# stevenmiller888/mlx-audio

Measured on AMD Instinct MI355X. Metric: audio-sec/sec (xRT), Kokoro-82M batch=32 fixed 128-phoneme utterances per GPU, higher is better.
Workload: dtype bf16; 1 GPU; Kokoro-82M bf16, batch=32/GPU fixed 128-phoneme utterances (T=130, F=650, 390000 samples = 16.25 s each), utterance-sharded over 1 GPU(s); global_batch=32, parallelism=utterance-shard x1, 2 batches in flight per GPU

## Files before the change

### mlx-audio_amd/csrc/kk_conv_mfma4.hip

```cpp
#include <stdlib.h>

#include "kk_common.h"
#include "kk_kernels.h"
#include "kk_conv_mfma_shared.h"

#define TR_NOW() 0ull
#define TR_ADD(slot, v) do { } while (0)
namespace {
typedef __bf16 bf16x2 __attribute__((ext_vector_type(2)));

typedef __bf16 bf16x8 __attribute__((ext_vector_type(8)));
typedef float f32x4 __attribute__((ext_vector_type(4)));

constexpr int BN = 128, CK = 64;
constexpr int XLD = 80;
constexpr int MAX_HALO = 50;
constexpr int CLD = BN;

constexpr int PS_BYTES = 2 * 3 * CK * 4;

template <int BM>
struct Geo {
  static constexpr int XROWS = BM + MAX_HALO;
  static constexpr int XS_BYTES = XROWS * XLD * 2;
  static constexpr int MAIN_BYTES = XS_BYTES + PS_BYTES;
  static constexpr int RPP = BM / 2;
  static constexpr int EPI_BYTES = RPP * CLD * 4;
  static constexpr int LDS_BYTES = MAIN_BYTES > EPI_BYTES ? MAIN_BYTES : EPI_BYTES;
  static constexpr int XREG = (XROWS * 8 + 255) / 256;
};


union U16 {
  uint4 u;
  bf16_t h[8];
};
union U32x8 {
  uint4 u[2];
  float f[8];
};

template <typename TO, int WM, int NRM>
__global__ __launch_bounds__(256, 2) __attribute__((amdgpu_waves_per_eu(2, 2))) void conv_mfma4_kernel(KKMfmaArgs a) {
  constexpr int BM = 2 * WM, MI16 = WM / 16;
  constexpr bool ACC16 = true;
  using G = Geo<BM>;
  constexpr int XREG = G::XREG;
  extern __shared__ __attribute__((aligned(16))) unsigned char smem[];
  bf16_t* Xs = (bf16_t*)smem;
  float* Ps = (float*)(smem + G::XS_BYTES);
  float* Cs = (float*)smem;

  const int tid = threadIdx.x, lane = tid & 63, wave = tid >> 6;
  const int wr = wave >> 1, wc = wave & 1;
  const int nphase = a.mode == KK_CONVT ? a.stride : 1;
  int bx, by, bz;
  {
    const int gx = gridDim.x, gy = gridDim.y, total = gx * gy * gridDim.z;
    int lid = blockIdx.x + gx * (blockIdx.y + gy * blockIdx.z);
    const int per = total / 8, rem = total - per * 8;
    const int xcd = lid & 7, idx = lid >> 3;
    lid = xcd * per + (xcd < rem ? xcd : rem) + idx;
    by = lid % gy;
    const int t = lid / gy;
    bx = t % gx;
    bz = t / gx;
  }
  const int b = bz / nphase, phase = bz - b * nphase;
  const int q0 = bx * BM, n0 = by * BN;
  const int Lin = kk_len(a.lin, b), Lout = kk_len(a.lout, b);

  int ntaps, off0, dstep, widx0, wstep;
  if (a.mode == KK_CONV) {
    ntaps = a.Kw; off0 = -a.pad; dstep = a.dil; widx0 = 0; wstep = 1;
  } else {
    const int k0 = (phase + a.pad) % a.stride;
    ntaps = (a.Kw - k0 + a.stride - 1) / a.stride;
    off0 = (phase + a.pad - k0) / a.stride; dstep = -1; widx0 = k0; wstep = a.stride;
  }
  const int min_off = dstep >= 0 ? off0 : off0 + (ntaps - 1) * dstep;
  const int halo = (ntaps - 1) * (dstep >= 0 ? dstep : -dstep);
  const int xrows = BM + halo;

  const int op_first = a.mode == KK_CONV ? q0 : phase + a.stride * q0;
  const bool tile_live = op_first < Lout;

  const unsigned long long tr0 = TR_NOW();
  unsigned long long tr_sx = 0, tr_sw = 0;
  (void)tr0; (void)tr_sx; (void)tr_sw;
  f32x4 acc[MI16][4];
#pragma unroll
  for (int i = 0; i < MI16; ++i)
#pragma unroll
    for (int j = 0; j < 4; ++j) acc[i][j] = f32x4{0.f, 0.f, 0.f, 0.f};

  if (tile_live) {
    const bf16_t* xb = a.x + (long long)b * a.xbs;
    const int nchunk = a.CinP / CK;
    const int nit = nchunk * ntaps;
    const int lin_hi = Lin > 0 ? Lin - 1 : 0;
    const int cin_real = a.Cin > 0 ? a.Cin : a.CinP;

#define KK_STG(name) name
#define KK_STG_XS Xs
#include "kk_conv_mfma_stage.h"
    uint4 q00, q01, q02, q03, q10, q11, q12, q13;
    const int nb = by;
    auto frag_ptr = [&](int it) __attribute__((always_inline)) -> const uint4* {
      const int chunk = it / ntaps, tap = it - chunk * ntaps;
      const long long blk = ((long long)(widx0 + tap * wstep) * (a.CoutP / BN) + nb) * nchunk + chunk;
      return (const uint4*)a.wf + blk * 1024 + (wc * 2) * 4 * 64 + lane;
    };
    load_x(0);
    {
      const uint4* fp = frag_ptr(0);
      q00 = fp[0 * 64]; q01 = fp[1 * 64]; q02 = fp[2 * 64]; q03 = fp[3 * 64];
      q10 = fp[4 * 64]; q11 = fp[5 * 64]; q12 = fp[6 * 64]; q13 = fp[7 * 64];
      asm volatile("" ::: "memory");
    }
    store_p(0);
    __syncthreads();
    store_x(0);
    __syncthreads();

    const int arow = wr * WM + (lane & 15);
    const int kofs = 8 * (lane >> 4);

    for (int it = 0; it < nit; ++it) {
      const int chunk = it / ntaps, tap = it - chunk * ntaps;
      const bool last_tap = tap == ntaps - 1;
      if (tap == 0 && chunk + 1 < nchunk) load_x(chunk + 1);
      const uint4* fn = frag_ptr(it + 1 < nit ? it + 1 : it);

      const int shift = (off0 + tap * dstep) - min_off;
      const bf16_t* xa = Xs + (arow + shift) * XLD + kofs;
      KK_MFMA_ITER(q00, q01, q02, q03, q10, q11, q12, q13)
      asm volatile("" ::: "memory");
      if (it + 1 < nit) {
        if (tap == 0 && chunk + 1 < nchunk) store_p(chunk + 1);
        if (last_tap) {
          __syncthreads();
          store_x(chunk + 1);
          __syncthreads();
        }
      }
    }
    __syncthreads();
  }

#include "kk_conv_mfma_epilogue.h"
}

template <int XR>
struct GeoWK {
  static constexpr int SROWS = XR == 7 ? 224 : 192 + MAX_HALO;
  static constexpr int SLAB = SROWS * XLD;
  static constexpr int XS_BYTES = 2 * SLAB * 2;
  static constexpr int MAIN_BYTES = XS_BYTES + PS_BYTES;
  static constexpr int RPP = 96;
  static constexpr int EPI_BYTES = RPP * CLD * 4;
  static constexpr int LDS_BYTES = MAIN_BYTES > EPI_BYTES ? MAIN_BYTES : EPI_BYTES;
};

template <int NRM, int XR>
__global__ __launch_bounds__(256, 2) __attribute__((amdgpu_waves_per_eu(2, 2))) void conv_mfma4_wholek_kernel(KKMfmaArgs a) {
  using TO = bf16_t;
  constexpr int WM = 96, BM = 2 * WM, MI16 = WM / 16, XREG = XR;
  constexpr bool ACC16 = true;
  using G = GeoWK<XR>;
  extern __shared__ __attribute__((aligned(16))) unsigned char smem[];
  bf16_t* Xs = (bf16_t*)smem;
  float* Ps = (float*)(smem + G::XS_BYTES);
  float* Cs = (float*)smem;

  const int tid = threadIdx.x, lane = tid & 63, wave = tid >> 6;
  const int wr = wave >> 1, wc = wave & 1;
  constexpr int nphase = 1, phase = 0;
  int bx, by, b;
  {
    const int gx = gridDim.x, gy = gridDim.y, total = gx * gy * gridDim.z;
    int lid = blockIdx.x + gx * (blockIdx.y + gy * blockIdx.z);
    const int per = total / 8, rem = total - per * 8;
    const int xcd = lid & 7, idx = lid >> 3;
    lid = xcd * per + (xcd < rem ? xcd : rem) + idx;
    by = lid % gy;
    const int t = lid / gy;
    bx = t % gx;
    b = t / gx;
  }
  const int q0 = bx * BM, n0 = by * BN;
  const int Lin = kk_len(a.lin, b), Lout = kk_len(a.lout, b);
  const int ntaps = a.Kw, off0 = -a.pad, dstep = a.dil, min_off = off0;
  const int xrows = BM + (ntaps - 1) * dstep;
  const bool tile_live = q0 < Lout;

  const unsigned long long tr0 = TR_NOW();
  (void)tr0;
  f32x4 acc[MI16][4];
#pragma unroll
  for (int i = 0; i < MI16; ++i)
#pragma unroll
    for (int j = 0; j < 4; ++j) acc[i][j] = f32x4{0.f, 0.f, 0.f, 0.f};

  if (tile_live) {
    const bf16_t* xb = a.x + (long long)b * a.xbs;
    const int nit = 2 * ntaps;
    const int lin_hi = Lin > 0 ? Lin - 1 : 0;
    const int cin_real = a.Cin > 0 ? a.Cin : a.CinP;

#define KK_STG(name) name##_s0
#define KK_STG_XS Xs
#include "kk_conv_mfma_stage.h"
#define KK_STG(name) name##_s1
#define KK_STG_XS (Xs + G::SLAB)
#include "kk_conv_mfma_stage.h"
    uint4 q00, q01, q02, q03, q10, q11, q12, q13;
    auto frag_ptr = [&](int it) __attribute__((always_inline)) -> const uint4* {
      const int chunk = it >= ntaps ? 1 : 0, tap = it - chunk * ntaps;
      const long long blk = ((long long)tap * (a.CoutP / BN) + by) * 2 + chunk;
      return (const uint4*)a.wf + blk * 1024 + (wc * 2) * 4 * 64 + lane;
    };
    load_x_s0(0);
    load_x_s1(1);
    {
      const uint4* fp = frag_ptr(0);
      q00 = fp[0 * 64]; q01 = fp[1 * 64]; q02 = fp[2 * 64]; q03 = fp[3 * 64];
      q10 = fp[4 * 64]; q11 = fp[5 * 64]; q12 = fp[6 * 64]; q13 = fp[7 * 64];
      asm volatile("" ::: "memory");
    }
    store_p_s0(0);
    store_p_s1(1);
    __syncthreads();
    store_x_s0(0);
    store_x_s1(1);
    __syncthreads();

    const int arow = wr * WM + (lane & 15);
    const int kofs = 8 * (lane >> 4);
    for (int it = 0; it + 1 < nit; ++it) {
      const int chunk = it >= ntaps ? 1 : 0, tap = it - chunk * ntaps;
      const uint4* fn = frag_ptr(it + 1);
      const bf16_t* xa = Xs + chunk * G::SLAB + (arow + tap * dstep) * XLD + kofs;
      KK_MFMA_ITER(q00, q01, q02, q03, q10, q11, q12, q13)
      asm volatile("" ::: "memory");
    }
    {
      const bf16_t* xa = Xs + G::SLAB + (arow + (ntaps - 1) * dstep) * XLD + kofs;
      KK_MFMA_ITER_LAST(q00, q01, q02, q03, q10, q11, q12, q13)
      asm volatile("" ::: "memory");
    }
    __syncthreads();
  }

#include "kk_conv_mfma_epilogue.h"
}

template <int NRM, int XR>
int launch_wholek(const KKMfmaArgs& a, int B, hipStream_t st) {
  using G = GeoWK<XR>;
  static KKDevOnce attr_once;
  if (attr_once.first()) {
    (void)hipFuncSetAttribute((const void*)conv_mfma4_wholek_kernel<NRM, XR>, hipFuncAttributeMaxDynamicSharedMemorySize, G::LDS_BYTES);
    attr_once.done();
  }
  dim3 grid(kk_cdiv(a.Q, 192), a.CoutP / BN, B);
  hipLaunchKernelGGL((conv_mfma4_wholek_kernel<NRM, XR>), grid, dim3(256), G::LDS_BYTES, st, a);
  KK_CHECK_LAUNCH();
  return 0;
}

template <typename TO, int WM, int NRM>
int launch_one(const KKMfmaArgs& a, int B, hipStream_t st) {
  using G = Geo<2 * WM>;
  static KKDevOnce attr_once;
  if (attr_once.first()) {
    (void)hipFuncSetAttribute((const void*)conv_mfma4_kernel<TO, WM, NRM>, hipFuncAttributeMaxDynamicSharedMemorySize, G::LDS_BYTES);
    attr_once.done();
  }
  const int nphase = a.mode == KK_CONVT ? a.stride : 1;
  dim3 grid(kk_cdiv(a.Q, 2 * WM), a.CoutP / BN, B * nphase);
  hipLaunchKernelGGL((conv_mfma4_kernel<TO, WM, NRM>), grid, dim3(256), G::LDS_BYTES, st, a);
  KK_CHECK_LAUNCH();
  return 0;
}

__global__ __launch_bounds__(256) void pack_w_frag_kernel(const bf16_t* w, bf16_t* wf, int Kw, int CoutP, int CinP) {
  const long long n = (long long)Kw * CoutP * CinP;
  for (long long e = (long long)blockIdx.x * 256 + threadIdx.x; e < n; e += (long long)gridDim.x * 256) {
    const int k = (int)(e % CinP);
    const long long r = e / CinP;
    const int cout = (int)(r % CoutP), tap = (int)(r / CoutP);
    wf[KK_MFMA4_PACK_INDEX(tap, cout, k, CoutP, CinP)] = w[e];
  }
}
}

int kk_launch_pack_w_frag(const void* w, void* wf, int Kw, int CoutP, int CinP, hipStream_t st) {
  if (CinP % CK != 0 || CoutP % BN != 0) return kk_fail("pack_w_frag: CinP must be a multiple of 64 and CoutP of 128");
  hipLaunchKernelGGL(pack_w_frag_kernel, dim3(1024), dim3(256), 0, st, (const bf16_t*)w, (bf16_t*)wf, Kw, CoutP, CinP);
  KK_CHECK_LAUNCH();
  return 0;
}

bool kk_mfma4_wholek_eligible(const KKMfmaArgs& a) {
  return a.mode == KK_CONV && a.stride == 1 && a.CinP == 2 * CK && a.dil >= 1 && (a.Kw - 1) * a.dil <= MAX_HALO;
}

int kk_launch_conv_mfma4(const KKMfmaArgs& a, int B, int out_dtype, hipStream_t st) {
  if (a.Q <= 0 || B <= 0) return 0;
  if (!a.wf) return kk_fail("conv_mfma4: fragment-order weights missing");
  const int nrm = a.nrm_a == nullptr ? 0 : (a.nrm_act == KK_ACT_SNAKE ? 1 : 2);
  if (nrm == 1 && a.nrm_C % 4 != 0) return kk_fail("conv_mfma: the fused Snake input needs a channel count that is a multiple of 4");
  KKMfmaArgs g = a;
  if (nrm == 2 && a.nrm_act != KK_ACT_LRELU) g.nrm_slope = 1.0f;
  if (out_dtype != KK_BF16) return kk_fail("conv_mfma4: bf16 output only");
  if (kk_mfma4_wholek_eligible(g) && !g.slabwise) {
    const bool x7 = (g.Kw - 1) * g.dil <= 32;
    if (nrm == 1) return x7 ? launch_wholek<1, 7>(g, B, st) : launch_wholek<1, 8>(g, B, st);
    if (nrm == 2) return x7 ? launch_wholek<2, 7>(g, B, st) : launch_wholek<2, 8>(g, B, st);
    return x7 ? launch_wholek<0, 7>(g, B, st) : launch_wholek<0, 8>(g, B, st);
  }
  if (nrm == 1) return launch_one<bf16_t, 96, 1>(g, B, st);
  if (nrm == 2) return launch_one<bf16_t, 96, 2>(g, B, st);
  return launch_one<bf16_t, 96, 0>(g, B, st);
}
```

### mlx-audio_amd/csrc/kk_conv_mfma_shared.h

```cpp
#pragma once
#include <hip/hip_runtime.h>

namespace {
struct v2f {
  float x, y;
};
__device__ __forceinline__ v2f operator*(v2f a, v2f b) { return v2f{a.x * b.x, a.y * b.y}; }
__device__ __forceinline__ v2f& operator+=(v2f& a, v2f b) { a.x += b.x; a.y += b.y; return a; }
__device__ __forceinline__ v2f& operator*=(v2f& a, v2f b) { a.x *= b.x; a.y *= b.y; return a; }
__device__ __forceinline__ v2f fma2(v2f a, v2f b, v2f c) { return v2f{__builtin_fmaf(a.x, b.x, c.x), __builtin_fmaf(a.y, b.y, c.y)}; }
__device__ __forceinline__ float gelu_exact(float v) { return 0.5f * v * (1.0f + erff(v * 0.70710678118654752440f)); }

typedef float kk_f32x4 __attribute__((ext_vector_type(4)));
typedef __bf16 kk_bf16x8 __attribute__((ext_vector_type(8)));

#define KK_MFMA_KSTEP(KS, B0, B1, B2, B3)                                                                                                  \
  {                                                                                                                                          \
    const kk_bf16x8 b0 = __builtin_bit_cast(kk_bf16x8, B0), b1 = __builtin_bit_cast(kk_bf16x8, B1);                                          \
    const kk_bf16x8 b2 = __builtin_bit_cast(kk_bf16x8, B2), b3 = __builtin_bit_cast(kk_bf16x8, B3);                                          \
    _Pragma("unroll") for (int mi = 0; mi < MI16; ++mi) {                                                                                    \
      const kk_bf16x8 av = *(const kk_bf16x8*)(xa + mi * 16 * XLD + (KS) * 32);                                                              \
      acc[mi][0] = __builtin_amdgcn_mfma_f32_16x16x32_bf16(av, b0, acc[mi][0], 0, 0, 0);                                                     \
      acc[mi][1] = __builtin_amdgcn_mfma_f32_16x16x32_bf16(av, b1, acc[mi][1], 0, 0, 0);                                                     \
      acc[mi][2] = __builtin_amdgcn_mfma_f32_16x16x32_bf16(av, b2, acc[mi][2], 0, 0, 0);                                                     \
      acc[mi][3] = __builtin_amdgcn_mfma_f32_16x16x32_bf16(av, b3, acc[mi][3], 0, 0, 0);                                                     \
    }                                                                                                                                        \
    B0 = fn[((KS) * 4 + 0) * 64];                                                                                                            \
    B1 = fn[((KS) * 4 + 1) * 64];                                                                                                            \
    B2 = fn[((KS) * 4 + 2) * 64];                                                                                                            \
    B3 = fn[((KS) * 4 + 3) * 64];                                                                                                            \
  }
#define KK_MFMA_ITER(Q00, Q01, Q02, Q03, Q10, Q11, Q12, Q13)                                                                               \
  KK_MFMA_KSTEP(0, Q00, Q01, Q02, Q03)                                                                                                     \
  KK_MFMA_KSTEP(1, Q10, Q11, Q12, Q13)                                                                                                     \
  __builtin_amdgcn_sched_group_barrier(0x100, 2, 0);                                                                                         \
  _Pragma("unroll") for (int ks = 0; ks < 2; ++ks) {                                                                                         \
    _Pragma("unroll") for (int j = 0; j < MI16; ++j) {                                                                                       \
      __builtin_amdgcn_sched_group_barrier(0x008, 4, 0);                                                                                     \
      if (ks * MI16 + j + 2 < 2 * MI16) __builtin_amdgcn_sched_group_barrier(0x100, 1, 0);                                                   \
    }                                                                                                                                        \
    __builtin_amdgcn_sched_group_barrier(0x020, 4, 0);                                                                                       \
  }
#define KK_MFMA_KSTEP_LAST(KS, B0, B1, B2, B3)                                                                                             \
  {                                                                                                                                          \
    const kk_bf16x8 b0 = __builtin_bit_cast(kk_bf16x8, B0), b1 = __builtin_bit_cast(kk_bf16x8, B1);                                          \
    const kk_bf16x8 b2 = __builtin_bit_cast(kk_bf16x8, B2), b3 = __builtin_bit_cast(kk_bf16x8, B3);                                          \
    _Pragma("unroll") for (int mi = 0; mi < MI16; ++mi) {                                                                                    \
      const kk_bf16x8 av = *(const kk_bf16x8*)(xa + mi * 16 * XLD + (KS) * 32);                                                              \
      acc[mi][0] = __builtin_amdgcn_mfma_f32_16x16x32_bf16(av, b0, acc[mi][0], 0, 0, 0);                                                     \
      acc[mi][1] = __builtin_amdgcn_mfma_f32_16x16x32_bf16(av, b1, acc[mi][1], 0, 0, 0);                                                     \
      acc[mi][2] = __builtin_amdgcn_mfma_f32_16x16x32_bf16(av, b2, acc[mi][2], 0, 0, 0);                                                     \
      acc[mi][3] = __builtin_amdgcn_mfma_f32_16x16x32_bf16(av, b3, acc[mi][3], 0, 0, 0);                                                     \
    }                                                                                                                                        \
  }
#define KK_MFMA_ITER_LAST(Q00, Q01, Q02, Q03, Q10, Q11, Q12, Q13)                                                                          \
  KK_MFMA_KSTEP_LAST(0, Q00, Q01, Q02, Q03)                                                                                                \
  KK_MFMA_KSTEP_LAST(1, Q10, Q11, Q12, Q13)                                                                                                \
  __builtin_amdgcn_sched_group_barrier(0x100, 2, 0);                                                                                         \
  _Pragma("unroll") for (int j = 0; j < 2 * MI16; ++j) {                                                                                     \
    __builtin_amdgcn_sched_group_barrier(0x008, 4, 0);                                                                                       \
    if (j + 2 < 2 * MI16) __builtin_amdgcn_sched_group_barrier(0x100, 1, 0);                                                                 \
  }
}
```

Measured before the change: 14700 audio-sec/sec.

## Prefetch LDS A-fragments across taps in a register ring, specialize 1-tap convs

Restructures the MFMA conv inner loops so A-operand LDS reads go into a small register ring (APF=3). The ring is primed before the loop and refilled for the next tap while the current tap's MFMAs run. Weight-fragment addresses are now advanced incrementally instead of being recomputed with divisions each iteration. A TAP1 template specialization gives kernel-size-1 convolutions a simpler chunk-only loop. The aim is to hide LDS latency and cut integer address arithmetic, at the cost of more VGPRs under the fixed two-waves-per-EU bound and some scheduling risk.

```diff
diff --git a/mlx-audio_amd/csrc/kk_conv_mfma4.hip b/mlx-audio_amd/csrc/kk_conv_mfma4.hip
--- a/mlx-audio_amd/csrc/kk_conv_mfma4.hip
+++ b/mlx-audio_amd/csrc/kk_conv_mfma4.hip
@@ -40,7 +40,7 @@
   float f[8];
 };
 
-template <typename TO, int WM, int NRM>
+template <typename TO, int WM, int NRM, bool TAP1>
 __global__ __launch_bounds__(256, 2) __attribute__((amdgpu_waves_per_eu(2, 2))) void conv_mfma4_kernel(KKMfmaArgs a) {
   constexpr int BM = 2 * WM, MI16 = WM / 16;
   constexpr bool ACC16 = true;
@@ -97,7 +97,6 @@
   if (tile_live) {
     const bf16_t* xb = a.x + (long long)b * a.xbs;
     const int nchunk = a.CinP / CK;
-    const int nit = nchunk * ntaps;
     const int lin_hi = Lin > 0 ? Lin - 1 : 0;
     const int cin_real = a.Cin > 0 ? a.Cin : a.CinP;
 
@@ -105,15 +104,12 @@
 #define KK_STG_XS Xs
 #include "kk_conv_mfma_stage.h"
     uint4 q00, q01, q02, q03, q10, q11, q12, q13;
-    const int nb = by;
-    auto frag_ptr = [&](int it) __attribute__((always_inline)) -> const uint4* {
-      const int chunk = it / ntaps, tap = it - chunk * ntaps;
-      const long long blk = ((long long)(widx0 + tap * wstep) * (a.CoutP / BN) + nb) * nchunk + chunk;
-      return (const uint4*)a.wf + blk * 1024 + (wc * 2) * 4 * 64 + lane;
-    };
+    const uint4* wslab = (const uint4*)a.wf + ((long long)widx0 * (a.CoutP / BN) + by) * nchunk * 1024;
+    const long long wtap = (long long)wstep * (a.CoutP / BN) * nchunk * 1024;
+    const unsigned wlane = (wc * 2) * 4 * 64 + lane;
     load_x(0);
     {
-      const uint4* fp = frag_ptr(0);
+      const uint4* fp = wslab + wlane;
       q00 = fp[0 * 64]; q01 = fp[1 * 64]; q02 = fp[2 * 64]; q03 = fp[3 * 64];
       q10 = fp[4 * 64]; q11 = fp[5 * 64]; q12 = fp[6 * 64]; q13 = fp[7 * 64];
       asm volatile("" ::: "memory");
@@ -123,22 +119,57 @@
     store_x(0);
     __syncthreads();
 
-    const int arow = wr * WM + (lane & 15);
-    const int kofs = 8 * (lane >> 4);
-
-    for (int it = 0; it < nit; ++it) {
-      const int chunk = it / ntaps, tap = it - chunk * ntaps;
-      const bool last_tap = tap == ntaps - 1;
-      if (tap == 0 && chunk + 1 < nchunk) load_x(chunk + 1);
-      const uint4* fn = frag_ptr(it + 1 < nit ? it + 1 : it);
-
-      const int shift = (off0 + tap * dstep) - min_off;
-      const bf16_t* xa = Xs + (arow + shift) * XLD + kofs;
-      KK_MFMA_ITER(q00, q01, q02, q03, q10, q11, q12, q13)
-      asm volatile("" ::: "memory");
-      if (it + 1 < nit) {
-        if (tap == 0 && chunk + 1 < nchunk) store_p(chunk + 1);
-        if (last_tap) {
+    const int xstep = dstep * XLD;
+    constexpr int APF = 3;
+    kk_bf16x8 apf[APF];
+    auto xa_first = [&]() __attribute__((always_inline)) -> const bf16_t* {
+      int t = tid;
+      asm volatile("" : "+v"(t));
+      return Xs + ((t >> 7) * WM + (t & 15) + (off0 - min_off)) * XLD + 8 * ((t & 63) >> 4);
+    };
+    if constexpr (TAP1) {
+      for (int chunk = 0; chunk < nchunk; ++chunk) {
+        const bool more = chunk + 1 < nchunk;
+        if (more) {
+          load_x(chunk + 1);
+          wslab += 1024;
+        }
+        const uint4* fn = wslab + wlane;
+        const bf16_t* xa = xa_first();
+        KK_MFMA_ITER(q00, q01, q02, q03, q10, q11, q12, q13)
+        asm volatile("" ::: "memory");
+        if (more) {
+          store_p(chunk + 1);
+          __syncthreads();
+          store_x(chunk + 1);
+          __syncthreads();
+        }
+      }
+    } else {
+      const uint4* wn = wslab;
+      for (int chunk = 0; chunk < nchunk; ++chunk) {
+        const bool more = chunk + 1 < nchunk;
+        if (more) load_x(chunk + 1);
+        const bf16_t* xa = xa_first();
+        KK_MFMA_PRIME(xa)
+        for (int tap = 0; tap + 1 < ntaps; ++tap) {
+          wn += wtap;
+          const uint4* fn = wn + wlane;
+          const bf16_t* xan = xa + xstep;
+          KK_MFMA_ITER_P(1, 1, q00, q01, q02, q03, q10, q11, q12, q13)
+          asm volatile("" ::: "memory");
+          xa = xan;
+          if (tap == 0 && more) store_p(chunk + 1);
+        }
+        {
+          if (more) { wslab += 1024; wn = wslab; }
+          const uint4* fn = wn + wlane;
+          const bf16_t* xan = nullptr;
+          (void)xan;
+          KK_MFMA_ITER_P(0, 1, q00, q01, q02, q03, q10, q11, q12, q13)
+          asm volatile("" ::: "memory");
+        }
+        if (more) {
           __syncthreads();
           store_x(chunk + 1);
           __syncthreads();
@@ -215,15 +246,13 @@
 #define KK_STG_XS (Xs + G::SLAB)
 #include "kk_conv_mfma_stage.h"
     uint4 q00, q01, q02, q03, q10, q11, q12, q13;
-    auto frag_ptr = [&](int it) __attribute__((always_inline)) -> const uint4* {
-      const int chunk = it >= ntaps ? 1 : 0, tap = it - chunk * ntaps;
-      const long long blk = ((long long)tap * (a.CoutP / BN) + by) * 2 + chunk;
-      return (const uint4*)a.wf + blk * 1024 + (wc * 2) * 4 * 64 + lane;
-    };
+    const uint4* const w0 = (const uint4*)a.wf + (long long)by * 2 * 1024;
+    const long long wtap = (long long)(a.CoutP / BN) * 2 * 1024;
+    const unsigned wlane = (wc * 2) * 4 * 64 + lane;
     load_x_s0(0);
     load_x_s1(1);
     {
-      const uint4* fp = frag_ptr(0);
+      const uint4* fp = w0 + wlane;
       q00 = fp[0 * 64]; q01 = fp[1 * 64]; q02 = fp[2 * 64]; q03 = fp[3 * 64];
       q10 = fp[4 * 64]; q11 = fp[5 * 64]; q12 = fp[6 * 64]; q13 = fp[7 * 64];
       asm volatile("" ::: "memory");
@@ -235,18 +264,30 @@
     store_x_s1(1);
     __syncthreads();
 
-    const int arow = wr * WM + (lane & 15);
-    const int kofs = 8 * (lane >> 4);
+    const bf16_t* const xa0 = Xs + (wr * WM + (lane & 15)) * XLD + 8 * (lane >> 4);
+    const int xstep = dstep * XLD;
+    constexpr int APF = 3;
+    kk_bf16x8 apf[APF];
+    const uint4* wn = w0;
+    const bf16_t* xa = xa0;
+    int xo = 0, tap = 0;
+    KK_MFMA_PRIME(xa)
     for (int it = 0; it + 1 < nit; ++it) {
-      const int chunk = it >= ntaps ? 1 : 0, tap = it - chunk * ntaps;
-      const uint4* fn = frag_ptr(it + 1);
-      const bf16_t* xa = Xs + chunk * G::SLAB + (arow + tap * dstep) * XLD + kofs;
-      KK_MFMA_ITER(q00, q01, q02, q03, q10, q11, q12, q13)
+      const bool wrap = ++tap == ntaps;
+      tap = wrap ? 0 : tap;
+      wn = wrap ? w0 + 1024 : wn + wtap;
+      xo = wrap ? G::SLAB : xo + xstep;
+      const uint4* fn = wn + wlane;
+      const bf16_t* xan = xa0 + xo;
+      KK_MFMA_ITER_P(1, 1, q00, q01, q02, q03, q10, q11, q12, q13)
       asm volatile("" ::: "memory");
+      xa = xan;
     }
     {
-      const bf16_t* xa = Xs + G::SLAB + (arow + (ntaps - 1) * dstep) * XLD + kofs;
-      KK_MFMA_ITER_LAST(q00, q01, q02, q03, q10, q11, q12, q13)
+      const uint4* fn = nullptr;
+      const bf16_t* xan = nullptr;
+      (void)fn; (void)xan;
+      KK_MFMA_ITER_P(0, 0, q00, q01, q02, q03, q10, q11, q12, q13)
       asm volatile("" ::: "memory");
     }
     __syncthreads();
@@ -269,19 +310,24 @@
   return 0;
 }
 
-template <typename TO, int WM, int NRM>
-int launch_one(const KKMfmaArgs& a, int B, hipStream_t st) {
+template <typename TO, int WM, int NRM, bool TAP1>
+int launch_one_t(const KKMfmaArgs& a, int B, hipStream_t st) {
   using G = Geo<2 * WM>;
   static KKDevOnce attr_once;
   if (attr_once.first()) {
-    (void)hipFuncSetAttribute((const void*)conv_mfma4_kernel<TO, WM, NRM>, hipFuncAttributeMaxDynamicSharedMemorySize, G::LDS_BYTES);
+    (void)hipFuncSetAttribute((const void*)conv_mfma4_kernel<TO, WM, NRM, TAP1>, hipFuncAttributeMaxDynamicSharedMemorySize, G::LDS_BYTES);
     attr_once.done();
   }
   const int nphase = a.mode == KK_CONVT ? a.stride : 1;
   dim3 grid(kk_cdiv(a.Q, 2 * WM), a.CoutP / BN, B * nphase);
-  hipLaunchKernelGGL((conv_mfma4_kernel<TO, WM, NRM>), grid, dim3(256), G::LDS_BYTES, st, a);
+  hipLaunchKernelGGL((conv_mfma4_kernel<TO, WM, NRM, TAP1>), grid, dim3(256), G::LDS_BYTES, st, a);
   KK_CHECK_LAUNCH();
   return 0;
+}
+
+template <typename TO, int WM, int NRM>
+int launch_one(const KKMfmaArgs& a, int B, hipStream_t st) {
+  return a.mode == KK_CONV && a.Kw == 1 ? launch_one_t<TO, WM, NRM, true>(a, B, st) : launch_one_t<TO, WM, NRM, false>(a, B, st);
 }
 
 __global__ __launch_bounds__(256) void pack_w_frag_kernel(const bf16_t* w, bf16_t* wf, int Kw, int CoutP, int CinP) {
diff --git a/mlx-audio_amd/csrc/kk_conv_mfma_shared.h b/mlx-audio_amd/csrc/kk_conv_mfma_shared.h
--- a/mlx-audio_amd/csrc/kk_conv_mfma_shared.h
+++ b/mlx-audio_amd/csrc/kk_conv_mfma_shared.h
@@ -41,24 +41,39 @@
     }                                                                                                                                        \
     __builtin_amdgcn_sched_group_barrier(0x020, 4, 0);                                                                                       \
   }
-#define KK_MFMA_KSTEP_LAST(KS, B0, B1, B2, B3)                                                                                             \
+
+#define KK_MFMA_PRIME(XA)                                                                                                                  \
+  static_assert(APF >= 1 && APF <= MI16 && (2 * MI16) % APF == 0, "the ring must come round at the end of an iteration");                  \
+  _Pragma("unroll") for (int g = 0; g < APF; ++g) apf[g] = *(const kk_bf16x8*)((XA) + g * 16 * XLD);
+#define KK_MFMA_KSTEP_P(KS, NEXT, REFILL, B0, B1, B2, B3)                                                                                  \
   {                                                                                                                                          \
     const kk_bf16x8 b0 = __builtin_bit_cast(kk_bf16x8, B0), b1 = __builtin_bit_cast(kk_bf16x8, B1);                                          \
     const kk_bf16x8 b2 = __builtin_bit_cast(kk_bf16x8, B2), b3 = __builtin_bit_cast(kk_bf16x8, B3);                                          \
     _Pragma("unroll") for (int mi = 0; mi < MI16; ++mi) {                                                                                    \
-      const kk_bf16x8 av = *(const kk_bf16x8*)(xa + mi * 16 * XLD + (KS) * 32);                                                              \
+      const int g = (KS) * MI16 + mi, gn = g + APF;                                                                                       \
+      const kk_bf16x8 av = apf[g % APF];                                                                                                  \
+      if (gn < 2 * MI16) apf[g % APF] = *(const kk_bf16x8*)(xa + (gn % MI16) * 16 * XLD + (gn / MI16) * 32);                              \
+      else if (NEXT) apf[g % APF] = *(const kk_bf16x8*)(xan + (gn - 2 * MI16) * 16 * XLD);                                                \
       acc[mi][0] = __builtin_amdgcn_mfma_f32_16x16x32_bf16(av, b0, acc[mi][0], 0, 0, 0);                                                     \
       acc[mi][1] = __builtin_amdgcn_mfma_f32_16x16x32_bf16(av, b1, acc[mi][1], 0, 0, 0);                                                     \
       acc[mi][2] = __builtin_amdgcn_mfma_f32_16x16x32_bf16(av, b2, acc[mi][2], 0, 0, 0);                                                     \
       acc[mi][3] = __builtin_amdgcn_mfma_f32_16x16x32_bf16(av, b3, acc[mi][3], 0, 0, 0);                                                     \
     }                                                                                                                                        \
+    if (REFILL) {                                                                                                                            \
+      B0 = fn[((KS) * 4 + 0) * 64];                                                                                                          \
+      B1 = fn[((KS) * 4 + 1) * 64];                                                                                                          \
+      B2 = fn[((KS) * 4 + 2) * 64];                                                                                                          \
+      B3 = fn[((KS) * 4 + 3) * 64];                                                                                                          \
+    }                                                                                                                                        \
   }
-#define KK_MFMA_ITER_LAST(Q00, Q01, Q02, Q03, Q10, Q11, Q12, Q13)                                                                          \
-  KK_MFMA_KSTEP_LAST(0, Q00, Q01, Q02, Q03)                                                                                                \
-  KK_MFMA_KSTEP_LAST(1, Q10, Q11, Q12, Q13)                                                                                                \
-  __builtin_amdgcn_sched_group_barrier(0x100, 2, 0);                                                                                         \
-  _Pragma("unroll") for (int j = 0; j < 2 * MI16; ++j) {                                                                                     \
-    __builtin_amdgcn_sched_group_barrier(0x008, 4, 0);                                                                                       \
-    if (j + 2 < 2 * MI16) __builtin_amdgcn_sched_group_barrier(0x100, 1, 0);                                                                 \
+#define KK_MFMA_ITER_P(NEXT, REFILL, Q00, Q01, Q02, Q03, Q10, Q11, Q12, Q13)                                                               \
+  KK_MFMA_KSTEP_P(0, NEXT, REFILL, Q00, Q01, Q02, Q03)                                                                                     \
+  KK_MFMA_KSTEP_P(1, NEXT, REFILL, Q10, Q11, Q12, Q13)                                                                                     \
+  _Pragma("unroll") for (int ks = 0; ks < 2; ++ks) {                                                                                         \
+    _Pragma("unroll") for (int j = 0; j < MI16; ++j) {                                                                                       \
+      __builtin_amdgcn_sched_group_barrier(0x008, 4, 0);                                                                                     \
+      if ((NEXT) || ks * MI16 + j + APF < 2 * MI16) __builtin_amdgcn_sched_group_barrier(0x100, 1, 0);                                    \
+    }                                                                                                                                        \
+    if (REFILL) __builtin_amdgcn_sched_group_barrier(0x020, 4, 0);                                                                           \
   }
 }
```

After: 14800 audio-sec/sec, median of 6. Within noise of the previous version (+0.7%).
